# aj-prime/Elemental

Hardware: AMD Instinct MI355X
Metric: distributed Gemm TFLOP/s (fp64/fp32) at 1/2/4/8 GPUs; % of MFMA peak (higher is better)
Workload: dtype f64; 1 GPU; C2: El::Gemm NN f64 m=n=k=32768, Grid 1x1; m=32768, n=32768, k=32768, grid=1x1, algorithm=SUMMA_C, blocksize=128, compute_panel=auto, parallelism=grid1x1, comm_reserved_cus=0

## Files before the change

### elemental_amd/_lib.py

```python
from __future__ import annotations

import ctypes
import os
from ctypes import (CFUNCTYPE, POINTER, c_char_p, c_double, c_float, c_int, c_int64, c_size_t,
                    c_ubyte, c_uint16, c_uint64, c_void_p)

_HERE = os.path.dirname(os.path.abspath(__file__))
LIB_PATH = os.path.join(_HERE, "libelemental_amd.so")

OK, ERR_LOGIC, ERR_HIP, ERR_COMM, ERR_RUNTIME, ERR_UNSUPPORTED, ERR_NO_DEVICE, ERR_SINGULAR = range(8)
ERR_NOT_HPD = 8
NORMAL, TRANSPOSE, ADJOINT = 0, 1, 2
MC, MD, MR, VC, VR, STAR, CIRC = range(7)
(GEMM_DEFAULT, GEMM_SUMMA_A_MS, GEMM_SUMMA_A, GEMM_SUMMA_B_MS, GEMM_SUMMA_B, GEMM_SUMMA_C_MS,
 GEMM_SUMMA_C, GEMM_SUMMA_DOT, GEMM_CANNON) = range(9)
ROW_MAJOR, COLUMN_MAJOR = 0, 1
LOWER, UPPER = 0, 1
LEFT, RIGHT = 0, 1
NON_UNIT, UNIT = 0, 1
CPU, GPU = 0, 1
F32, F64, F16, BF16 = 0, 1, 2, 3
I32, I64, U8 = 4, 5, 6
OP_SUM, OP_PROD, OP_MAX, OP_MIN = 0, 1, 2, 3
(MAP_IDENTITY, MAP_NEGATE, MAP_ABS, MAP_SQUARE, MAP_SQRT, MAP_EXP, MAP_LOG, MAP_RELU, MAP_SIGMOID,
# ... 11 lines not shown
    "elx_last_error": (c_char_p, []),
    "elx_last_nonhpd_column": (_i, []),
    "elx_version": (_i, []),
    "elx_device_count": (_i, [POINTER(c_int)]),
    "elx_set_device": (_i, [_i]),
    "elx_get_device": (_i, [POINTER(c_int)]),
    "elx_device_synchronize": (_i, []),
    "elx_default_stream": (_i, [POINTER(c_void_p)]),
    "elx_comm_stream": (_i, [POINTER(c_void_p)]),
    "elx_reserved_cus": (_i, [POINTER(c_int)]),
    "elx_stream_create": (_i, [POINTER(c_void_p)]),
    "elx_stream_destroy": (_i, [_vp]),
    "elx_stream_synchronize": (_i, [_vp]),
    "elx_default_event": (_i, [POINTER(c_void_p)]),
    "elx_event_create": (_i, [POINTER(c_void_p)]),
    "elx_event_destroy": (_i, [_vp]),
    "elx_event_record": (_i, [_vp, _vp]),
    "elx_stream_wait_event": (_i, [_vp, _vp]),
    "elx_event_synchronize": (_i, [_vp]),
    "elx_pool_alloc": (_i, [POINTER(c_void_p), c_size_t, _vp]),
    "elx_pool_free": (_i, [_vp, _vp]),
    "elx_pool_trim": (_i, [c_size_t]),
    "elx_pool_stats": (_i, [POINTER(c_size_t), POINTER(c_size_t)]),
    "elx_pool_set_max_cached": (_i, [c_size_t]),
    "elx_pool_max_cached": (_i, [POINTER(c_size_t)]),
    "elx_pool_bin_bytes": (c_size_t, [c_size_t]),
    "elx_pool_bin_cacheable": (_i, [c_size_t]),
    "elx_pool_backing_reserved": (_i, [POINTER(c_size_t)]),
    "elx_memcpy_h2d": (_i, [_vp, _vp, c_size_t, _vp]),
    "elx_memcpy_d2h": (_i, [_vp, _vp, c_size_t, _vp]),
    "elx_memcpy_d2d": (_i, [_vp, _vp, c_size_t, _vp]),
    "elx_gemm_f64": (_i, [_i, _i, _i64, _i64, _i64, _d, _vp, _i64, _vp, _i64, _d, _vp, _i64, _vp]),
    "elx_gemm_f32": (_i, [_i, _i, _i64, _i64, _i64, c_float, _vp, _i64, _vp, _i64, c_float, _vp, _i64, _vp]),
    "elx_gemm_f16": (_i, [_i, _i, _i64, _i64, _i64, c_float, _vp, _i64, _vp, _i64, c_float, _vp, _i64, _vp]),
    "elx_gemm_bf16": (_i, [_i, _i, _i64, _i64, _i64, c_float, _vp, _i64, _vp, _i64, c_float, _vp, _i64, _vp]),
    "elx_matrix_gemm": (_i, [_i, _i, _i, _i, _i64, _i64, _i64, _d, _vp, _i64, _vp, _i64, _d, _vp, _i64, _vp]),
    "elx_matrix_fill": (_i, [_i, _i, _i64, _i64, _d, _vp, _i64, _vp]),
    "elx_matrix_scale": (_i, [_i, _i, _i64, _i64, _d, _vp, _i64, _vp]),
    "elx_matrix_axpy": (_i, [_i, _i, _i64, _i64, _d, _vp, _i64, _vp, _i64, _vp]),
    "elx_matrix_copy": (_i, [_i, _i, _i64, _i64, _vp, _i64, _vp, _i64, _vp]),
    "elx_matrix_trmm": (_i, [_i, _i, _i, _i, _i, _i, _i64, _i64, _d, _vp, _i64, _vp, _i64, _vp]),
    "elx_matrix_trsm": (_i, [_i, _i, _i, _i, _i, _i, _i64, _i64, _d, _vp, _i64, _vp, _i64, _vp]),
    "elx_trsm_plan": (_i, [_i, _i64, _i64, POINTER(c_int), POINTER(c_int), POINTER(c_int64)]),
    "elx_trsm_last_launch": (_i, []),
    "elx_matrix_cholesky": (_i, [_i, _i, _i, _i64, _vp, _i64, _vp]),
    "elx_matrix_triangular_inverse": (_i, [_i, _i, _i, _i, _i64, _vp, _i64, _vp]),
    "elx_matrix_trtrmm": (_i, [_i, _i, _i, _i64, _vp, _i64, _vp]),
    "elx_matrix_hpd_inverse": (_i, [_i, _i, _i, _i64, _vp, _i64, _vp]),
    "elx_matrix_lu": (_i, [_i, _i, _i64, _i64, _vp, _i64, _vp, _vp]),
    "elx_matrix_qr": (_i, [_i, _i, _i64, _i64, _vp, _i64, _vp, _vp, _vp]),
    "elx_matrix_hermitian_tridiag": (_i, [_i, _i, _i, _i64, _vp, _i64, _vp, _vp]),
    "elx_axpy2d": (_i, [_i, _i64, _i64, _d, _vp, _i64, _i64, _vp, _i64, _i64, _vp]),
    "elx_copy2d": (_i, [_i, _i64, _i64, _vp, _i64, _i64, _vp, _i64, _i64, _vp]),
    "elx_pack_strided": (_i, [_i, _i, _i64, _i64, _i64, _i64, _i64, _i64, _vp, _i64, _vp, _i64, _vp]),
    "elx_unpack_strided": (_i, [_i, _i, _i64, _i64, _i64, _i64, _i64, _i64, _vp, _i64, _vp, _i64, _vp]),
    "elx_pack_partial_strided": (_i, [_i, _i, _i, _i64, _i64, _i64, _i64, _i64, _i64, _i64, _i64, _vp, _i64, _vp,
                                      _i64, _vp]),
    "elx_unpack_partial_strided": (_i, [_i, _i, _i, _i64, _i64, _i64, _i64, _i64, _i64, _i64, _i64, _vp, _i64,
                                        _vp, _i64, _vp]),
    "elx_unpack_axpy_strided": (_i, [_i, _i, _i64, _i64, _d, _i64, _i64, _i64, _i64, _vp, _i64, _vp, _i64, _vp]),
    "elx_copy2d_convert": (_i, [_i, _i, _i64, _i64, _vp, _i64, _i64, _vp, _i64, _i64, _vp]),
    "elx_transpose": (_i, [_i, _i64, _i64, _vp, _i64, _vp, _i64, _vp]),
    "elx_scale2d": (_i, [_i, _i64, _i64, _d, _vp, _i64, _vp]),
    "elx_fill2d": (_i, [_i, _i64, _i64, _d, _vp, _i64, _vp]),
    "elx_hadamard2d": (_i, [_i, _i64, _i64, _vp, _i64, _vp, _i64, _vp, _i64, _vp]),
    "elx_entrywise_map": (_i, [_i, _i, _i64, _i64, _vp, _i64, _vp, _i64, _vp]),
# ... 214 lines not shown
```

### elemental_amd/csrc/capi.cpp

```cpp
#include "common.hpp"
#include "runtime/runtime.hpp"
#include "comm/comm.hpp"
#include "core/distmatrix.hpp"
#include "core/redist.hpp"
#include "core/gemm.hpp"
#include "core/level2.hpp"
#include "core/lu.hpp"
#include "core/qr.hpp"
#include "core/tridiag.hpp"
#include "core/random.hpp"
#include "core/io.hpp"
#include "core/exec.hpp"
#include <functional>
#include <string>

struct elx_comm_s { std::shared_ptr<elx::Comm> c; };
struct elx_grid_s { std::shared_ptr<elx::Grid> g; };
struct elx_dm_s { std::shared_ptr<elx::DistMatrix> m; };
struct elx_perm_s { elx::Permutation p; };

namespace elx {
namespace {
thread_local std::string g_last_error;

// ... 124 lines not shown
}
int elx_memcpy_d2h(void* dst, const void* src, size_t bytes, void* stream) {
    return Guard([&] {
        hipStream_t s = S(stream);
        ELX_CHECK_HIP(hipMemcpyAsync(dst, src, bytes, hipMemcpyDeviceToHost, s));
        ELX_CHECK_HIP(hipStreamSynchronize(s));
    });
}
int elx_memcpy_d2d(void* dst, const void* src, size_t bytes, void* stream) {
    return Guard([&] { ELX_CHECK_HIP(hipMemcpyAsync(dst, src, bytes, hipMemcpyDeviceToDevice, S(stream))); });
}

#define ELX_GEMM_ENTRY(NAME, DT, ST, SC)                                                              \
    int NAME(int opA, int opB, int64_t m, int64_t n, int64_t k, SC alpha, const ST* A, int64_t lda,    \
             const ST* B, int64_t ldb, SC beta, ST* C, int64_t ldc, void* stream) {                  \
        return Guard([&] {                                                                             \
            CheckOp(opA);                                                                              \
            CheckOp(opB);                                                                              \
            ELX_REQUIRE(m >= 0 && n >= 0 && k >= 0, "negative GEMM dimension");                       \
            const bool ta = opA != ELX_NORMAL, tb = opB != ELX_NORMAL;                                 \
            ELX_REQUIRE(ldc >= (m > 1 ? m : 1), "ldc too small");                                     \
            ELX_REQUIRE(lda >= ((ta ? k : m) > 1 ? (ta ? k : m) : 1), "lda too small");               \
            ELX_REQUIRE(ldb >= ((tb ? n : k) > 1 ? (tb ? n : k) : 1), "ldb too small");               \
            if (m == 0 || n == 0) return;                                                              \
            exec::Gemm(Device::GPU, DT, ta, tb, m, n, k, (double)alpha, A, lda, B, ldb, (double)beta, C, \
                       ldc, S(stream));                                                                \
        });                                                                                            \
    }
ELX_GEMM_ENTRY(elx_gemm_f64, DType::F64, double, double)
ELX_GEMM_ENTRY(elx_gemm_f32, DType::F32, float, float)
ELX_GEMM_ENTRY(elx_gemm_f16, DType::F16, uint16_t, float)
ELX_GEMM_ENTRY(elx_gemm_bf16, DType::BF16, uint16_t, float)
#undef ELX_GEMM_ENTRY

namespace {
hipStream_t DevStream(Device d, void* stream) { return d == Device::GPU ? S(stream) : nullptr; }
void CheckLd(int64_t ld, int64_t rows, const char* what) {
    ELX_REQUIRE(ld >= (rows > 1 ? rows : 1), what, " leading dimension ", ld, " < ", rows);
}
}
int elx_matrix_gemm(int dtype, int device, int opA, int opB, int64_t m, int64_t n, int64_t k, double alpha,
                    const void* A, int64_t lda, const void* B, int64_t ldb, double beta, void* C, int64_t ldc,
                    void* stream) {
    return Guard([&] {
        CheckOp(opA);
        CheckOp(opB);
        ELX_REQUIRE(m >= 0 && n >= 0 && k >= 0, "negative GEMM dimension");
        const bool ta = opA != ELX_NORMAL, tb = opB != ELX_NORMAL;
        CheckLd(ldc, m, "C");
        CheckLd(lda, ta ? k : m, "A");
        CheckLd(ldb, tb ? n : k, "B");
        if (m == 0 || n == 0) return;
        const Device d = ToDevice(device);
        if (k == 0) {
            if (beta == 0.0) exec::Fill(d, ToDType(dtype), m, n, 0.0, C, ldc, DevStream(d, stream));
            else if (beta != 1.0) exec::Scale(d, ToDType(dtype), m, n, beta, C, ldc, DevStream(d, stream));
            return;
        }
        exec::Gemm(d, ToDType(dtype), ta, tb, m, n, k, alpha, A, lda, B, ldb, beta, C, ldc, DevStream(d, stream));
    });
}
int elx_matrix_fill(int dtype, int device, int64_t m, int64_t n, double value, void* A, int64_t lda, void* stream) {
    return Guard([&] {
        CheckLd(lda, m, "A");
        if (m == 0 || n == 0) return;
        const Device d = ToDevice(device);
// ... 972 lines not shown
```

### elemental_amd/csrc/core/exec.cpp

```cpp
#include <cstdlib>
#include "exec.hpp"
#include "host_blas.hpp"
#include "host_leaves.hpp"
#include <cmath>
#include <type_traits>
#include <vector>

namespace elx {
namespace exec {

namespace {

[[noreturn]] void NotAMatrixType(DType t) { throw LogicError(Cat("dtype ", DTypeName(t), " is not a matrix type")); }
#define EXEC_SWITCH(t, T, ...) ELX_DTYPE_SWITCH(t, T, NotAMatrixType(t), __VA_ARGS__)
#define EXEC_REAL_SWITCH(t, T, ...) ELX_REAL_SWITCH(t, T, NotAMatrixType(t), __VA_ARGS__)

void check(hipError_t e, const char* what) {
    if (e != hipSuccess)
        throw HIPError(Cat(what, ": ", hipGetErrorName(e), " (", hipGetErrorString(e), ")"));
}

}

int CommCopyWGs() {
    static const int v = [] { const char* e = getenv("ELX_COMM_COPY_WGS"); return e ? atoi(e) : 256; }();
    return v;
}

void Copy2DBatch(Device dev, DType t, const Copy2D* d, int nd, bool axpy, double alpha, hipStream_t s) {
    if (nd <= 0) return;
    if (dev == Device::GPU) {
        const int cap = s != nullptr && s == Runtime::Get().CommStream() ? CommCopyWGs() : 0;
        check(kern::copy2d_batch(static_cast<int>(t), d, nd, axpy, alpha, s, cap), "copy2d_batch");
        return;
// ... 5 lines not shown
                 int nsrc, double alpha, hipStream_t s) {
    if (m <= 0 || n <= 0 || nsrc <= 0) return;
    if (dev == Device::GPU) {
        const int cap = s != nullptr && s == Runtime::Get().CommStream() ? CommCopyWGs() : 0;
        for (int q0 = 0; q0 < nsrc; q0 += kern::kMaxContractSources) {
            kern::ContractSum c{};
            c.m = m; c.n = n; c.dst = dst; c.dcs = dcs; c.drs = drs;
            c.nsrc = std::min(nsrc - q0, kern::kMaxContractSources);
            for (int q = 0; q < c.nsrc; ++q) {
                c.src[q] = src[q0 + q].p;
                c.scs[q] = src[q0 + q].cs;
                c.srs[q] = src[q0 + q].rs;
            }
            check(kern::contract_sum(static_cast<int>(t), c, alpha, s, cap), "contract_sum");
        }
        return;
    }
    for (int q = 0; q < nsrc; ++q) {
        const Copy2D d{m, n, src[q].p, src[q].cs, src[q].rs, dst, dcs, drs};
        EXEC_SWITCH(t, T, cpu_copy<T>(d, true, alpha));
    }
}

void Convert2D(Device dev, DType src_t, DType dst_t, const Copy2D& d, hipStream_t s) {
    if (d.m <= 0 || d.n <= 0) return;
    if (src_t == dst_t) { Copy2DBatch(dev, src_t, &d, 1, false, 0.0, s); return; }
    if (dev == Device::GPU) {
        check(kern::convert2d(static_cast<int>(src_t), static_cast<int>(dst_t), d, s), "convert2d");
        return;
    }
    EXEC_SWITCH(src_t, TS, EXEC_SWITCH(dst_t, TD, cpu_convert<TS, TD>(d)));
}

void Gemm(Device dev, DType t, bool ta, bool tb, Int m, Int n, Int k, double alpha, const void* A, Int lda,
          const void* B, Int ldb, double beta, void* C, Int ldc, hipStream_t s) {
    if (m <= 0 || n <= 0) return;
    if (dev == Device::GPU) {
        hipError_t e = hipSuccess;
        switch (t) {
        case DType::F64:
            e = kern::gemm_mfma<double>(ta, tb, m, n, k, alpha, static_cast<const double*>(A), lda,
                                        static_cast<const double*>(B), ldb, beta, static_cast<double*>(C), ldc, s);
            break;
        case DType::F32:
            e = kern::gemm_mfma<float>(ta, tb, m, n, k, (float)alpha, static_cast<const float*>(A), lda,
                                       static_cast<const float*>(B), ldb, (float)beta, static_cast<float*>(C),
                                       ldc, s);
            break;
        case DType::F16:
        case DType::BF16:
            e = kern::gemm_mfma_h(t == DType::BF16, ta, tb, m, n, k, (float)alpha,
                                  static_cast<const uint16_t*>(A), lda, static_cast<const uint16_t*>(B), ldb,
                                  (float)beta, static_cast<uint16_t*>(C), ldc, s);
            break;
        default:
            NotAMatrixType(t);
        }
        check(e, "gemm_mfma");
        return;
    }
    EXEC_SWITCH(t, T,
        cpu_gemm<T>(ta, tb, m, n, k, alpha, static_cast<const Stor<T>*>(A), lda, static_cast<const Stor<T>*>(B), ldb,
                    beta, static_cast<Stor<T>*>(C), ldc));
}

void Fill(Device dev, DType t, Int m, Int n, double v, void* A, Int lda, hipStream_t s) {
    if (m <= 0 || n <= 0) return;
    if (dev == Device::GPU) { check(kern::fill2d((int)t, m, n, v, A, lda, s), "fill2d"); return; }
// ... 390 lines not shown
```

### elemental_amd/csrc/core/exec.hpp

```cpp
#pragma once
#include "../common.hpp"
#include "../runtime/runtime.hpp"
#include "../kernels/kernels.hpp"

namespace elx {
namespace exec {

using kern::Copy2D;

void Copy2DBatch(Device dev, DType t, const Copy2D* d, int nd, bool axpy, double alpha, hipStream_t s);
struct ContractSource { const void* p; Int cs, rs; };
void ContractSum(Device dev, DType t, Int m, Int n, void* dst, Int dcs, Int drs, const ContractSource* src,
                 int nsrc, double alpha, hipStream_t s);
void Convert2D(Device dev, DType src_t, DType dst_t, const Copy2D& d, hipStream_t s);
void Gemm(Device dev, DType t, bool ta, bool tb, Int m, Int n, Int k, double alpha,
          const void* A, Int lda, const void* B, Int ldb, double beta, void* C, Int ldc, hipStream_t s);
void Fill(Device dev, DType t, Int m, Int n, double v, void* A, Int lda, hipStream_t s);
void Scale(Device dev, DType t, Int m, Int n, double alpha, void* A, Int lda, hipStream_t s);
double AbsMax(Device dev, DType t, Int m, Int n, const void* A, Int lda, hipStream_t s);
double ScaledSumSq(Device dev, DType t, Int m, Int n, const void* A, Int lda, double scale, hipStream_t s);
void Hadamard(Device dev, DType t, Int m, Int n, const void* A, Int lda, const void* B, Int ldb,
              void* C, Int ldc, hipStream_t s);
void Map(Device dev, DType t, int fn, Int m, Int n, const void* A, Int lda, void* B, Int ldb, hipStream_t s);
void Combine(Device dev, DType t, int fn, Int m, Int n, const void* A, Int lda, void* B, Int ldb, hipStream_t s);
void Trapezoid(Device dev, DType t, bool lower, Int m, Int n, double alpha, const void* X, Int ldx, double beta,
               void* Y, Int ldy, Int i0, Int is, Int j0, Int js, Int offset, hipStream_t s);
void Trsm(Device dev, DType t, bool lower, bool trans, bool unit, Int m, Int n, const void* A, Int lda, void* B,
          Int ldb, hipStream_t s);
void Trmm(Device dev, DType t, bool lower, bool trans, bool unit, Int m, Int n, double alpha, const void* A, Int lda,
          void* B, Int ldb, hipStream_t s);
void Cholesky(Device dev, DType t, bool lower, Int n, void* A, Int lda, int* info, int col0, hipStream_t s);
size_t LUWorkBytes(Device dev, Int m);
void LU(Device dev, DType t, Int m, Int w, void* A, Int lda, int* piv, int row_off, void* work, int* info, int col0,
        hipStream_t s);
void Laswp(Device dev, DType t, Int m, Int n, void* A, Int lda, const int* piv, Int k0, Int k1, Int voff, bool inverse,
           const int* info, hipStream_t s);
size_t QRWorkBytes(Device dev, Int m);
void QR(Device dev, DType t, Int m, Int w, void* A, Int lda, void* tau, void* sig, void* work, hipStream_t s);
void QRExplicitU(Device dev, DType t, Int m, Int nb, const void* A, Int lda, void* U, Int ldu, hipStream_t s,
                 bool upper = false, Int off = 0);
size_t SytrdWorkBytes(Int n);
void SytrdPanel(DType t, bool lower, Int n, Int c0, Int w, void* A, Int lda, void* tau, void* V, void* W, Int ldv,
                void* work, hipStream_t s);
void HostHermitianTridiag(DType t, bool lower, Int n, void* A, Int lda, void* tau);
void QRFixT(Device dev, DType t, Int nb, void* S, Int lds, const void* tau, hipStream_t s);
void RowScale(Device dev, DType t, Int m, Int n, void* A, Int lda, const void* sig, Int i0, Int is, hipStream_t s);
void TriangularInverse(Device dev, DType t, bool lower, bool unit, Int n, void* A, Int lda, hipStream_t s);
void Trtrmm(Device dev, DType t, bool lower, Int n, void* A, Int lda, hipStream_t s);
void TriInverseBatched(DType t, bool lower, bool trans, bool unit, Int nb, Int m, const void* A, Int lda, void* W,
// ... 22 lines not shown
```

### elemental_amd/csrc/kernels/blas1.hip

```cpp
#include <hip/hip_runtime.h>
#include "kernels.hpp"
#include "dtype_switch.hpp"
#include <algorithm>
#include <cstdlib>
#include <initializer_list>
#include <utility>

namespace elx {
namespace kern {

namespace {

constexpr int TILE = 64;
constexpr int NT = 256;
constexpr int UNROLL = 4;

struct CopyBatch {
    Copy2D d[kMaxCopyBatch];
};

template <typename S>
struct V16 {
    static constexpr int N = 16 / sizeof(S);
    S v[N];
// ... 453 lines not shown
                      [&](const S(&x)[2]) { return E::store(apply_combine(FN, E::load(x[1]), E::load(x[0]))); });
}

template <typename T>
__global__ __launch_bounds__(NT) void hash_kernel(i64 m, i64 n, typename Elem<T>::storage* A, i64 lda, i64 i0,
                                                  i64 istride, i64 j0, i64 jstride, uint64_t seed,
                                                  double center, double radius) {
    using E = Elem<T>;
    for_each_2d(m, n, [&](i64 i, i64 j) {
#pragma clang fp contract(off)
        const double u = hash_unit(seed, i0 + i * istride, j0 + j * jstride);
        const double v = center + radius * (2.0 * u - 1.0);
        A[i + j * lda] = E::store((typename E::compute)v);
    });
}

template <typename T>
__global__ __launch_bounds__(NT) void trapezoid_kernel(bool lower, i64 m, i64 n, double alpha,
                                                       const typename Elem<T>::storage* X, i64 ldx, double beta,
                                                       typename Elem<T>::storage* Y, i64 ldy, i64 i0, i64 istride,
                                                       i64 j0, i64 jstride, i64 offset) {
    using E = Elem<T>;
    using Cm = typename E::compute;
    const Cm a = (Cm)alpha, b = (Cm)beta;
    for_each_2d(m, n, [&](i64 i, i64 j) {
        const i64 gi = i0 + i * istride, gj = j0 + j * jstride - offset;
        if (lower ? gi < gj : gi > gj) return;
        Cm y = (X && beta == 0.0) ? Cm(0) : b * E::load(Y[i + j * ldy]);
        if (X) y = y + a * E::load(X[i + j * ldx]);
        Y[i + j * ldy] = E::store(y);
    });
}

struct EwShape {
    i64 m, n;
    bool vec;
    dim3 grid;
};
template <typename S>
EwShape ew_shape(i64 m, i64 n, std::initializer_list<std::pair<const void*, i64>> ops) {
    bool contig = true, vec = true;
    for (auto& o : ops) {
        contig = contig && (o.second == m || n == 1);
        vec = vec && (reinterpret_cast<uintptr_t>(o.first) % 16 == 0);
    }
    if (contig) { m *= n; n = 1; }
    for (auto& o : ops) vec = vec && (n == 1 || (o.second * (i64)sizeof(S)) % 16 == 0);
    constexpr int N = 16 / sizeof(S);
    i64 gx = (m + (i64)NT * N * UNROLL - 1) / ((i64)NT * N * UNROLL);
    const i64 gy = n < 1 ? 1 : (n > 65535 ? 65535 : n);
    gx = std::max<i64>(1, std::min<i64>(gx, (1ll << 31) - 1));
    return EwShape{m, n, vec, dim3((unsigned)gx, (unsigned)gy)};
}

dim3 grid2d(i64 m, i64 n) {
    i64 gx = (m + NT - 1) / NT;
    if (gx > 64) gx = 64;
    if (gx < 1) gx = 1;
    i64 gy = n < 1 ? 1 : n;
    if (gy > 4096) gy = 4096;
    return dim3((unsigned)gx, (unsigned)gy);
}

bool TransposeVec(const Copy2D& x, int es) {
    const bool src_i = x.scs == 1, dst_i = x.dcs == 1;
    if (src_i == dst_i || (src_i ? false : x.srs != 1) || (dst_i ? false : x.drs != 1)) return false;
// ... 203 lines not shown
hipError_t combine(int dtype, int fn, i64 m, i64 n, const void* A, i64 lda, void* B, i64 ldb, hipStream_t s) {
    if (m <= 0 || n <= 0) return hipSuccess;
#define ELX_COMBINE_CASE(F) case F: launch_combine<T, F>(s, m, n, A, lda, B, ldb); break;
    ELX_KERN_SWITCH(dtype, T, switch (fn) {
        ELX_COMBINE_CASE(ELX_COMBINE_ADD) ELX_COMBINE_CASE(ELX_COMBINE_SUB) ELX_COMBINE_CASE(ELX_COMBINE_MUL)
        ELX_COMBINE_CASE(ELX_COMBINE_DIV) ELX_COMBINE_CASE(ELX_COMBINE_MAX) ELX_COMBINE_CASE(ELX_COMBINE_MIN)
        ELX_COMBINE_CASE(ELX_COMBINE_RELU_GRAD)
        default: return hipErrorInvalidValue;
    });
#undef ELX_COMBINE_CASE
    return hipGetLastError();
}

hipError_t fill_hash(int dtype, i64 m, i64 n, void* A, i64 lda, i64 i0, i64 istride, i64 j0, i64 jstride,
                     uint64_t seed, double center, double radius, hipStream_t s) {
    if (m <= 0 || n <= 0) return hipSuccess;
    ELX_KERN_SWITCH(dtype, T,
        hipLaunchKernelGGL((hash_kernel<T>), grid2d(m, n), dim3(NT), 0, s, m, n,
                           static_cast<typename Elem<T>::storage*>(A), lda, i0, istride, j0, jstride,
                           seed, center, radius));
    return hipGetLastError();
}

hipError_t trapezoid2d(int dtype, bool lower, i64 m, i64 n, double alpha, const void* X, i64 ldx, double beta,
                       void* Y, i64 ldy, i64 i0, i64 istride, i64 j0, i64 jstride, i64 offset, hipStream_t s) {
    if (m <= 0 || n <= 0) return hipSuccess;
    ELX_KERN_SWITCH(dtype, T,
        hipLaunchKernelGGL((trapezoid_kernel<T>), grid2d(m, n), dim3(NT), 0, s, lower, m, n, alpha,
                           static_cast<const typename Elem<T>::storage*>(X), ldx, beta,
                           static_cast<typename Elem<T>::storage*>(Y), ldy, i0, istride, j0, jstride, offset));
    return hipGetLastError();
}

}
}
```

### elemental_amd/csrc/kernels/kernels.hpp

```cpp
#pragma once
#include <hip/hip_runtime.h>
#include <algorithm>
#include <cstdint>
#include <cstdlib>

namespace elx {
namespace kern {

hipError_t workspace_alloc(void** p, size_t bytes, hipStream_t s);
hipError_t workspace_free(void* p, hipStream_t s);

using i64 = int64_t;

template <typename T>
hipError_t gemm_mfma(bool ta, bool tb, i64 m, i64 n, i64 k, T alpha, const T* A, i64 lda,
                     const T* B, i64 ldb, T beta, T* C, i64 ldc, hipStream_t s);
struct DmaPlan {
    bool use;
    i64 kmain, kchunk;
    int nz;
};
inline DmaPlan dma_plan(bool ok, i64 tiles, i64 k, int bk, i64 slots = 512) {
    DmaPlan d{false, 0, 0, 1};
    if (!ok) return d;
// ... 85 lines not shown
        const i64 z = std::min<i64>(std::min<i64>((256 + tiles - 1) / tiles, kmain / (min_kt * BK)), split_cap);
        if (z >= 2) {
            pl.kchunk = ((kmain + z - 1) / z + BK - 1) / BK * BK;
            pl.nz = (kmain + pl.kchunk - 1) / pl.kchunk;
        }
    }
    return pl;
}

hipError_t gemm_mfma_h(bool is_bf16, bool ta, bool tb, i64 m, i64 n, i64 k, float alpha,
                       const uint16_t* A, i64 lda, const uint16_t* B, i64 ldb, float beta,
                       uint16_t* C, i64 ldc, hipStream_t s);
hipError_t gemm_mfma_h_simple(bool is_bf16, bool ta, bool tb, i64 m, i64 n, i64 k, float alpha,
                              const uint16_t* A, i64 lda, const uint16_t* B, i64 ldb, float beta,
                              uint16_t* C, i64 ldc, hipStream_t s);

struct Copy2D {
    i64 m, n;
    const void* src; i64 scs, srs;
    void* dst; i64 dcs, drs;
};
constexpr int kMaxCopyBatch = 16;
hipError_t copy2d_batch(int dtype, const Copy2D* d, int nd, bool axpy, double alpha, hipStream_t s, int max_wgs = 0);

constexpr int kMaxContractSources = 16;
struct ContractSum {
    i64 m, n;
    void* dst; i64 dcs, drs;
    int nsrc;
    const void* src[kMaxContractSources];
    i64 scs[kMaxContractSources], srs[kMaxContractSources];
};
hipError_t contract_sum(int dtype, const ContractSum& c, double alpha, hipStream_t s, int max_wgs = 0);

hipError_t convert2d(int src_dtype, int dst_dtype, const Copy2D& d, hipStream_t s);
hipError_t fill2d(int dtype, i64 m, i64 n, double v, void* A, i64 lda, hipStream_t s);
constexpr int kNormPartsMax = 4096;
hipError_t norm_partials(int dtype, int mode, i64 m, i64 n, const void* A, i64 lda, double scale, double* out,
                         int* nparts, hipStream_t s);
hipError_t scale2d(int dtype, i64 m, i64 n, double alpha, void* A, i64 lda, hipStream_t s);
hipError_t hadamard2d(int dtype, i64 m, i64 n, const void* A, i64 lda, const void* B, i64 ldb,
                      void* C, i64 ldc, hipStream_t s);
hipError_t entrywise_map(int dtype, int fn, i64 m, i64 n, const void* A, i64 lda, void* B, i64 ldb,
                         hipStream_t s);
hipError_t combine(int dtype, int fn, i64 m, i64 n, const void* A, i64 lda, void* B, i64 ldb, hipStream_t s);
hipError_t fill_hash(int dtype, i64 m, i64 n, void* A, i64 lda, i64 i0, i64 istride, i64 j0,
                     i64 jstride, uint64_t seed, double center, double radius, hipStream_t s);

hipError_t trapezoid2d(int dtype, bool lower, i64 m, i64 n, double alpha, const void* X, i64 ldx, double beta,
                       void* Y, i64 ldy, i64 i0, i64 istride, i64 j0, i64 jstride, i64 offset, hipStream_t s);
hipError_t trsm_local(int dtype, bool ident, bool lower, bool trans, bool unit, i64 m, i64 n, const void* A, i64 lda,
                      void* B, i64 ldb, hipStream_t s);
constexpr long kTriInverseLdsMax = 150 * 1024;
bool tri_inverse_lds_ok(int dtype, i64 nb);
hipError_t tri_inverse_batched(int dtype, bool lower, bool trans, bool unit, i64 nb, i64 m, const void* A, i64 lda,
                               void* W, hipStream_t s);
constexpr i64 kTrsmInvertMaxRows = 256;
constexpr long kTrsmLdsMax = 66 * 1024;
struct TrsmPlan { bool invert; bool lds; size_t lds_bytes; };
constexpr TrsmPlan trsm_plan(size_t es, i64 m, i64 n) {
    const size_t bytes = (size_t)m * 65 * es;
    return TrsmPlan{m <= kTrsmInvertMaxRows && n >= 4 * m, bytes <= (size_t)kTrsmLdsMax, bytes};
}
constexpr bool trsm_batched_ok(size_t es, i64 nb, i64 m, i64 local_width) {
    return nb * 65 * (i64)es <= kTriInverseLdsMax && (m + nb - 1) / nb <= 65535 && local_width >= 4 * nb;
}
// ... 51 lines not shown
```

### include/elemental_amd.h

```cpp
#ifndef ELEMENTAL_AMD_H
#define ELEMENTAL_AMD_H

#include <stddef.h>
#include <stdint.h>

#ifdef __cplusplus
extern "C" {
#endif

#define ELX_OK                  0
#define ELX_ERR_LOGIC           1
#define ELX_ERR_HIP             2
#define ELX_ERR_COMM            3
#define ELX_ERR_RUNTIME         4
#define ELX_ERR_UNSUPPORTED     5
#define ELX_ERR_NO_DEVICE       6
#define ELX_ERR_SINGULAR        7
#define ELX_ERR_NOT_HPD         8

#define ELX_NORMAL     0
#define ELX_TRANSPOSE  1
#define ELX_ADJOINT    2
#define ELX_MC    0
#define ELX_MD    1
// ... 58 lines not shown
int elx_comm_stream(void** stream);
int elx_reserved_cus(int* cus);
int elx_stream_create(void** stream);
int elx_stream_destroy(void* stream);
int elx_stream_synchronize(void* stream);
int elx_default_event(void** event);
int elx_event_create(void** event);
int elx_event_destroy(void* event);
int elx_event_record(void* event, void* stream);
int elx_stream_wait_event(void* stream, void* event);
int elx_event_synchronize(void* event);

int elx_pool_alloc(void** ptr, size_t bytes, void* stream);
int elx_pool_free(void* ptr, void* stream);
int elx_pool_trim(size_t bytes_to_keep);
int elx_pool_stats(size_t* bytes_reserved, size_t* bytes_in_use);
int elx_pool_set_max_cached(size_t bytes);
int elx_pool_max_cached(size_t* bytes);
size_t elx_pool_bin_bytes(size_t bytes);
int elx_pool_bin_cacheable(size_t bytes);
int elx_pool_backing_reserved(size_t* bytes);
int elx_memcpy_h2d(void* dst, const void* src, size_t bytes, void* stream);
int elx_memcpy_d2h(void* dst, const void* src, size_t bytes, void* stream);
int elx_memcpy_d2d(void* dst, const void* src, size_t bytes, void* stream);

int elx_gemm_f64(int opA, int opB, int64_t m, int64_t n, int64_t k,
                 double alpha, const double* A, int64_t lda,
                 const double* B, int64_t ldb,
                 double beta, double* C, int64_t ldc, void* stream);
int elx_gemm_f32(int opA, int opB, int64_t m, int64_t n, int64_t k,
                 float alpha, const float* A, int64_t lda,
                 const float* B, int64_t ldb,
                 float beta, float* C, int64_t ldc, void* stream);
int elx_gemm_f16(int opA, int opB, int64_t m, int64_t n, int64_t k,
                 float alpha, const uint16_t* A, int64_t lda,
                 const uint16_t* B, int64_t ldb,
                 float beta, uint16_t* C, int64_t ldc, void* stream);
int elx_gemm_bf16(int opA, int opB, int64_t m, int64_t n, int64_t k,
                  float alpha, const uint16_t* A, int64_t lda,
                  const uint16_t* B, int64_t ldb,
                  float beta, uint16_t* C, int64_t ldc, void* stream);

int elx_matrix_gemm(int dtype, int device, int opA, int opB, int64_t m, int64_t n, int64_t k,
                    double alpha, const void* A, int64_t lda, const void* B, int64_t ldb,
                    double beta, void* C, int64_t ldc, void* stream);
int elx_matrix_fill(int dtype, int device, int64_t m, int64_t n, double value,
                    void* A, int64_t lda, void* stream);
int elx_matrix_scale(int dtype, int device, int64_t m, int64_t n, double alpha,
                     void* A, int64_t lda, void* stream);
int elx_matrix_axpy(int dtype, int device, int64_t m, int64_t n, double alpha,
                    const void* X, int64_t ldx, void* Y, int64_t ldy, void* stream);
int elx_matrix_copy(int dtype, int device, int64_t m, int64_t n, const void* A, int64_t lda,
                    void* B, int64_t ldb, void* stream);
int elx_matrix_trmm(int dtype, int device, int side, int uplo, int orient, int diag,
                    int64_t m, int64_t n, double alpha, const void* A, int64_t lda,
                    void* B, int64_t ldb, void* stream);
int elx_matrix_trsm(int dtype, int device, int side, int uplo, int orient, int diag,
                    int64_t m, int64_t n, double alpha, const void* A, int64_t lda,
                    void* B, int64_t ldb, void* stream);
int elx_trsm_plan(int dtype, int64_t m, int64_t n, int* invert, int* lds, int64_t* lds_bytes);
int elx_trsm_last_launch(void);
int elx_matrix_cholesky(int dtype, int device, int uplo, int64_t n, void* A, int64_t lda, void* stream);
int elx_matrix_triangular_inverse(int dtype, int device, int uplo, int diag, int64_t n, void* A, int64_t lda,
                                  void* stream);
int elx_matrix_trtrmm(int dtype, int device, int uplo, int64_t n, void* A, int64_t lda, void* stream);
int elx_matrix_hpd_inverse(int dtype, int device, int uplo, int64_t n, void* A, int64_t lda, void* stream);
// ... 256 lines not shown
```

Before: 76.32 TFLOP/s.

## Add one-level Strassen recursion for large f32/f64 GEMMs

Routes eligible f32/f64 GEMMs (all dims even and at least 8192, nonzero alpha, GPU) through a Strassen-Winograd recursion, one level by default and configurable via environment variables. It replaces eight half-size multiplies with seven, plus new fused quadrant-sum and quadrant-scatter kernels. The aim is to cut MFMA work by about one eighth in exchange for extra memory-bound additions, three half-size workspace buffers, and weaker floating-point error bounds compared with classical GEMM.

New measurement: 86.03 TFLOP/s, median of 6. +12.7%, better.

```diff
diff --git a/elemental_amd/_lib.py b/elemental_amd/_lib.py
--- a/elemental_amd/_lib.py
+++ b/elemental_amd/_lib.py
@@ -67,6 +67,7 @@
     "elx_memcpy_d2d": (_i, [_vp, _vp, c_size_t, _vp]),
     "elx_gemm_f64": (_i, [_i, _i, _i64, _i64, _i64, _d, _vp, _i64, _vp, _i64, _d, _vp, _i64, _vp]),
     "elx_gemm_f32": (_i, [_i, _i, _i64, _i64, _i64, c_float, _vp, _i64, _vp, _i64, c_float, _vp, _i64, _vp]),
+    "elx_gemm_last_levels": (_i, []),
     "elx_gemm_f16": (_i, [_i, _i, _i64, _i64, _i64, c_float, _vp, _i64, _vp, _i64, c_float, _vp, _i64, _vp]),
     "elx_gemm_bf16": (_i, [_i, _i, _i64, _i64, _i64, c_float, _vp, _i64, _vp, _i64, c_float, _vp, _i64, _vp]),
     "elx_matrix_gemm": (_i, [_i, _i, _i, _i, _i64, _i64, _i64, _d, _vp, _i64, _vp, _i64, _d, _vp, _i64, _vp]),
diff --git a/elemental_amd/csrc/capi.cpp b/elemental_amd/csrc/capi.cpp
--- a/elemental_amd/csrc/capi.cpp
+++ b/elemental_amd/csrc/capi.cpp
@@ -180,6 +180,7 @@
 ELX_GEMM_ENTRY(elx_gemm_f16, DType::F16, uint16_t, float)
 ELX_GEMM_ENTRY(elx_gemm_bf16, DType::BF16, uint16_t, float)
 #undef ELX_GEMM_ENTRY
+int elx_gemm_last_levels(void) { return exec::GemmLastLevels(); }
 
 namespace {
 hipStream_t DevStream(Device d, void* stream) { return d == Device::GPU ? S(stream) : nullptr; }
diff --git a/elemental_amd/csrc/core/exec.cpp b/elemental_amd/csrc/core/exec.cpp
--- a/elemental_amd/csrc/core/exec.cpp
+++ b/elemental_amd/csrc/core/exec.cpp
@@ -1,5 +1,6 @@
 #include <cstdlib>
 #include "exec.hpp"
+#include "strassen.hpp"
 #include "host_blas.hpp"
 #include "host_leaves.hpp"
 #include <cmath>
@@ -71,8 +72,56 @@
     EXEC_SWITCH(src_t, TS, EXEC_SWITCH(dst_t, TD, cpu_convert<TS, TD>(d)));
 }
 
+namespace {
+thread_local int t_gemm_levels = 0;
+}
+int GemmLastLevels() { return t_gemm_levels; }
+
 void Gemm(Device dev, DType t, bool ta, bool tb, Int m, Int n, Int k, double alpha, const void* A, Int lda,
           const void* B, Int ldb, double beta, void* C, Int ldc, hipStream_t s) {
+    t_gemm_levels = 0;
+    if (m <= 0 || n <= 0) return;
+    if (k >= 2 && (t == DType::F64 || t == DType::F32)) {
+        const strassen::Knobs kn = strassen::ReadKnobs();
+        t_gemm_levels = strassen::Gemm(kn.levels, kn, dev, t, ta, tb, m, n, k, alpha, A, lda, B, ldb, beta, C, ldc, s);
+        if (t_gemm_levels > 0) return;
+    }
+    GemmPlain(dev, t, ta, tb, m, n, k, alpha, A, lda, B, ldb, beta, C, ldc, s);
+}
+
+void QuadSum(Device dev, DType t, const kern::QuadSum* q, int nq, hipStream_t s) {
+    RequireReal(t, "QuadSum");
+    if (dev == Device::GPU) { check(kern::quad_sum((int)t, q, nq, s), "quad_sum"); return; }
+    for (int d = 0; d < nq; ++d)
+        EXEC_REAL_SWITCH(t, T, {
+            const kern::QuadSum& a = q[d];
+            const T* x = static_cast<const T*>(a.x);
+            const T* y = static_cast<const T*>(a.y);
+            T* o = static_cast<T*>(a.d);
+            for (Int j = 0; j < a.n; ++j)
+                for (Int i = 0; i < a.m; ++i) o[i + j * a.ldd] = x[i + j * a.ldx] + (T)a.sy * y[i + j * a.ldy];
+        });
+}
+
+void QuadScatter(Device dev, DType t, const kern::QuadScatter& q, hipStream_t s) {
+    RequireReal(t, "QuadScatter");
+    if (dev == Device::GPU) { check(kern::quad_scatter((int)t, q, s), "quad_scatter"); return; }
+    EXEC_REAL_SWITCH(t, T, {
+        const T* M = static_cast<const T*>(q.M);
+        for (int w = 0; w < q.nt; ++w) {
+            T* c = static_cast<T*>(q.c[w]);
+            for (Int j = 0; j < q.n; ++j)
+                for (Int i = 0; i < q.m; ++i) {
+                    T v = (T)q.coef[w] * M[i + j * q.ldm];
+                    if (q.beta[w] != 0.0) v = v + (T)q.beta[w] * c[i + j * q.ldc[w]];
+                    c[i + j * q.ldc[w]] = v;
+                }
+        }
+    });
+}
+
+void GemmPlain(Device dev, DType t, bool ta, bool tb, Int m, Int n, Int k, double alpha, const void* A, Int lda,
+               const void* B, Int ldb, double beta, void* C, Int ldc, hipStream_t s) {
     if (m <= 0 || n <= 0) return;
     if (dev == Device::GPU) {
         hipError_t e = hipSuccess;
diff --git a/elemental_amd/csrc/core/exec.hpp b/elemental_amd/csrc/core/exec.hpp
--- a/elemental_amd/csrc/core/exec.hpp
+++ b/elemental_amd/csrc/core/exec.hpp
@@ -15,6 +15,11 @@
 void Convert2D(Device dev, DType src_t, DType dst_t, const Copy2D& d, hipStream_t s);
 void Gemm(Device dev, DType t, bool ta, bool tb, Int m, Int n, Int k, double alpha,
           const void* A, Int lda, const void* B, Int ldb, double beta, void* C, Int ldc, hipStream_t s);
+void GemmPlain(Device dev, DType t, bool ta, bool tb, Int m, Int n, Int k, double alpha,
+               const void* A, Int lda, const void* B, Int ldb, double beta, void* C, Int ldc, hipStream_t s);
+int GemmLastLevels();
+void QuadSum(Device dev, DType t, const kern::QuadSum* q, int nq, hipStream_t s);
+void QuadScatter(Device dev, DType t, const kern::QuadScatter& q, hipStream_t s);
 void Fill(Device dev, DType t, Int m, Int n, double v, void* A, Int lda, hipStream_t s);
 void Scale(Device dev, DType t, Int m, Int n, double alpha, void* A, Int lda, hipStream_t s);
 double AbsMax(Device dev, DType t, Int m, Int n, const void* A, Int lda, hipStream_t s);
diff --git a/elemental_amd/csrc/core/strassen.cpp b/elemental_amd/csrc/core/strassen.cpp
--- /dev/null
+++ b/elemental_amd/csrc/core/strassen.cpp
@@ -0,0 +1,107 @@
+#include "strassen.hpp"
+#include "exec.hpp"
+#include <cstdlib>
+
+namespace elx {
+namespace strassen {
+
+Knobs ReadKnobs() {
+    Knobs kn{1, kDefaultMin, false};
+    if (const char* v = getenv("ELX_GEMM_STRASSEN")) kn.levels = std::max(0, std::min(2, atoi(v)));
+    if (const char* v = getenv("ELX_GEMM_STRASSEN_MIN")) {
+        kn.min = std::max<Int>(2, atoll(v));
+        kn.forced = true;
+    }
+    return kn;
+}
+
+bool Eligible(Device dev, DType t, Int m, Int n, Int k, double alpha, const Knobs& kn) {
+    if (t != DType::F64 && t != DType::F32) return false;
+    if (dev != Device::GPU && !kn.forced) return false;
+    if ((m | n | k) & 1) return false;
+    return std::min(m, std::min(n, k)) >= kn.min && alpha != 0.0;
+}
+
+namespace {
+
+struct Work {
+    Device dev;
+    hipStream_t s;
+    void* p = nullptr;
+    Work(Device d, hipStream_t st) : dev(d), s(st) {}
+    Work(const Work&) = delete;
+    Work& operator=(const Work&) = delete;
+    bool Alloc(size_t bytes) {
+        if (dev == Device::GPU) return kern::workspace_alloc(&p, bytes, s) == hipSuccess && p != nullptr;
+        p = std::malloc(bytes);
+        return p != nullptr;
+    }
+    ~Work() {
+        if (!p) return;
+        if (dev == Device::GPU) (void)kern::workspace_free(p, s);
+        else std::free(p);
+    }
+};
+
+int Multiply(int levels, const Knobs& kn, Device dev, DType t, bool ta, bool tb, Int m, Int n, Int k, double alpha,
+             const void* A, Int lda, const void* B, Int ldb, double beta, void* C, Int ldc, hipStream_t s) {
+    const int used = Gemm(levels, kn, dev, t, ta, tb, m, n, k, alpha, A, lda, B, ldb, beta, C, ldc, s);
+    if (used == 0) exec::GemmPlain(dev, t, ta, tb, m, n, k, alpha, A, lda, B, ldb, beta, C, ldc, s);
+    return used;
+}
+
+}
+
+int Gemm(int levels, const Knobs& kn, Device dev, DType t, bool ta, bool tb, Int m, Int n, Int k, double alpha,
+         const void* A, Int lda, const void* B, Int ldb, double beta, void* C, Int ldc, hipStream_t s) {
+    if (levels <= 0 || !Eligible(dev, t, m, n, k, alpha, kn)) return 0;
+    const Int m2 = m / 2, n2 = n / 2, k2 = k / 2;
+    const size_t es = DTypeSize(t);
+    const Int ra = ta ? k2 : m2, ca = ta ? m2 : k2, rb = tb ? n2 : k2, cb = tb ? k2 : n2;
+    Work Sw(dev, s), Tw(dev, s), Mw(dev, s);
+    if (!Sw.Alloc((size_t)ra * ca * es) || !Tw.Alloc((size_t)rb * cb * es) || !Mw.Alloc((size_t)m2 * n2 * es)) return 0;
+    void* S = Sw.p;
+    void* T = Tw.p;
+    void* M = Mw.p;
+
+    const char* a = static_cast<const char*>(A);
+    const char* b = static_cast<const char*>(B);
+    char* c = static_cast<char*>(C);
+    auto Aq = [&](int p, int q) -> const void* { return a + (ta ? q * k2 + p * m2 * lda : p * m2 + q * k2 * lda) * (Int)es; };
+    auto Bq = [&](int p, int q) -> const void* { return b + (tb ? q * n2 + p * k2 * ldb : p * k2 + q * n2 * ldb) * (Int)es; };
+    auto Cq = [&](int p, int q) -> void* { return c + (p * m2 + q * n2 * ldc) * (Int)es; };
+
+    auto sums = [&](const void* X, Int ldx, const void* Y, Int ldy, double sx, const void* V, Int ldv, const void* W,
+                    Int ldw, double sv) {
+        const kern::QuadSum q[2] = {{ra, ca, S, ra, X, ldx, Y, ldy, sx}, {rb, cb, T, rb, V, ldv, W, ldw, sv}};
+        exec::QuadSum(dev, t, q, 2, s);
+    };
+    auto scatter = [&](int nt, void* c0, double beta0, void* c1, double beta1) {
+        const kern::QuadScatter q{m2, n2, M, m2, nt, {c0, c1}, {ldc, ldc}, {beta0, beta1}, {alpha, alpha}};
+        exec::QuadScatter(dev, t, q, s);
+    };
+    int deep = 0;
+    auto mul = [&](double al, const void* X, Int ldx, const void* Y, Int ldy, double be, void* Z, Int ldz) {
+        deep = std::max(deep, Multiply(levels - 1, kn, dev, t, ta, tb, m2, n2, k2, al, X, ldx, Y, ldy, be, Z, ldz, s));
+    };
+
+    sums(Aq(1, 0), lda, Aq(1, 1), lda, 1.0, Bq(0, 1), ldb, Bq(0, 0), ldb, -1.0);
+    mul(1.0, S, ra, T, rb, 0.0, M, m2);
+    scatter(2, Cq(0, 1), beta, Cq(1, 1), beta);
+    sums(S, ra, Aq(0, 0), lda, -1.0, Bq(1, 1), ldb, T, rb, -1.0);
+    mul(1.0, Aq(0, 0), lda, Bq(0, 0), ldb, 0.0, M, m2);
+    scatter(1, Cq(0, 0), beta, nullptr, 0.0);
+    mul(alpha, Aq(0, 1), lda, Bq(1, 0), ldb, 1.0, Cq(0, 0), ldc);
+    mul(1.0, S, ra, T, rb, 1.0, M, m2);
+    sums(Aq(0, 1), lda, S, ra, -1.0, T, rb, Bq(1, 0), ldb, -1.0);
+    mul(alpha, S, ra, Bq(1, 1), ldb, 1.0, Cq(0, 1), ldc);
+    mul(-alpha, Aq(1, 1), lda, T, rb, beta, Cq(1, 0), ldc);
+    scatter(1, Cq(0, 1), 1.0, nullptr, 0.0);
+    sums(Aq(0, 0), lda, Aq(1, 0), lda, -1.0, Bq(1, 1), ldb, Bq(0, 1), ldb, -1.0);
+    mul(1.0, S, ra, T, rb, 1.0, M, m2);
+    scatter(2, Cq(1, 0), 1.0, Cq(1, 1), 1.0);
+    return 1 + deep;
+}
+
+}
+}
diff --git a/elemental_amd/csrc/core/strassen.hpp b/elemental_amd/csrc/core/strassen.hpp
--- /dev/null
+++ b/elemental_amd/csrc/core/strassen.hpp
@@ -0,0 +1,24 @@
+#pragma once
+#include "../common.hpp"
+#include "../runtime/runtime.hpp"
+
+namespace elx {
+namespace strassen {
+
+constexpr Int kMinFloor = 8192;
+constexpr Int kDefaultMin = kMinFloor;
+
+struct Knobs {
+    int levels;
+    Int min;
+    bool forced;
+};
+Knobs ReadKnobs();
+
+bool Eligible(Device dev, DType t, Int m, Int n, Int k, double alpha, const Knobs& kn);
+
+int Gemm(int levels, const Knobs& kn, Device dev, DType t, bool ta, bool tb, Int m, Int n, Int k, double alpha,
+         const void* A, Int lda, const void* B, Int ldb, double beta, void* C, Int ldc, hipStream_t s);
+
+}
+}
diff --git a/elemental_amd/csrc/kernels/blas1.hip b/elemental_amd/csrc/kernels/blas1.hip
--- a/elemental_amd/csrc/kernels/blas1.hip
+++ b/elemental_amd/csrc/kernels/blas1.hip
@@ -509,6 +509,95 @@
     });
 }
 
+struct QuadSumBatch {
+    QuadSum q[2];
+};
+
+template <typename T>
+__global__ __launch_bounds__(NT) void quad_sum_kernel(QuadSumBatch b, bool vec) {
+    using E = Elem<T>;
+    using S = typename E::storage;
+    const QuadSum& q = b.q[blockIdx.z];
+    const auto sy = (typename E::compute)q.sy;
+    S* const p[3] = {static_cast<S*>(q.d), const_cast<S*>(static_cast<const S*>(q.x)),
+                     const_cast<S*>(static_cast<const S*>(q.y))};
+    const i64 l[3] = {q.ldd, q.ldx, q.ldy};
+    ew_2d<S, 3, false>(q.m, q.n, p, l, vec, [&](const S(&x)[3]) { return E::store(E::load(x[1]) + sy * E::load(x[2])); });
+}
+
+template <typename T>
+__global__ __launch_bounds__(NT) void quad_scatter_kernel(QuadScatter q, bool vec) {
+    using E = Elem<T>;
+    using S = typename E::storage;
+    using Cm = typename E::compute;
+    constexpr int N = V16<S>::N;
+    constexpr i64 CHUNK = (i64)NT * UNROLL * N;
+    const S* M = static_cast<const S*>(q.M);
+    S* const c0p = static_cast<S*>(q.c[0]);
+    S* const c1p = static_cast<S*>(q.c[1]);
+    const bool two = q.nt > 1;
+    const bool rd0 = q.beta[0] != 0.0, rd1 = two && q.beta[1] != 0.0;
+    const Cm b0 = (Cm)q.beta[0], b1 = (Cm)q.beta[1], a0 = (Cm)q.coef[0], a1 = (Cm)q.coef[1];
+    auto out = [](Cm a, S mv, bool rd, Cm b, S cv) {
+        Cm v = a * E::load(mv);
+        if (rd) v = v + b * E::load(cv);
+        return E::store(v);
+    };
+    for (i64 j = blockIdx.y; j < q.n; j += gridDim.y) {
+        const S* mc = M + j * q.ldm;
+        S* y0 = c0p + j * q.ldc[0];
+        S* y1 = two ? c1p + j * q.ldc[1] : nullptr;
+        for (i64 c0 = (i64)blockIdx.x * CHUNK; c0 < q.m; c0 += (i64)gridDim.x * CHUNK) {
+            if (vec && c0 + CHUNK <= q.m) {
+                V16<S> x[UNROLL], u0[UNROLL] = {}, u1[UNROLL] = {};
+#pragma unroll
+                for (int u = 0; u < UNROLL; ++u) {
+                    const i64 i = c0 + (u * NT + threadIdx.x) * N;
+                    x[u] = *reinterpret_cast<const V16<S>*>(mc + i);
+                    if (rd0) u0[u] = *reinterpret_cast<const V16<S>*>(y0 + i);
+                    if (rd1) u1[u] = *reinterpret_cast<const V16<S>*>(y1 + i);
+                }
+#pragma unroll
+                for (int u = 0; u < UNROLL; ++u) {
+                    const i64 i = c0 + (u * NT + threadIdx.x) * N;
+#pragma unroll
+                    for (int e = 0; e < N; ++e) u0[u].v[e] = out(a0, x[u].v[e], rd0, b0, u0[u].v[e]);
+                    *reinterpret_cast<V16<S>*>(y0 + i) = u0[u];
+                    if (two) {
+#pragma unroll
+                        for (int e = 0; e < N; ++e) u1[u].v[e] = out(a1, x[u].v[e], rd1, b1, u1[u].v[e]);
+                        *reinterpret_cast<V16<S>*>(y1 + i) = u1[u];
+                    }
+                }
+            } else {
+                const i64 end = c0 + CHUNK < q.m ? c0 + CHUNK : q.m;
+                for (i64 i = c0 + (i64)threadIdx.x * N; i < end; i += (i64)NT * N) {
+                    if (vec && i + N <= end) {
+                        const V16<S> x = *reinterpret_cast<const V16<S>*>(mc + i);
+                        V16<S> u0 = {}, u1 = {};
+                        if (rd0) u0 = *reinterpret_cast<const V16<S>*>(y0 + i);
+                        if (rd1) u1 = *reinterpret_cast<const V16<S>*>(y1 + i);
+#pragma unroll
+                        for (int e = 0; e < N; ++e) u0.v[e] = out(a0, x.v[e], rd0, b0, u0.v[e]);
+                        *reinterpret_cast<V16<S>*>(y0 + i) = u0;
+                        if (two) {
+#pragma unroll
+                            for (int e = 0; e < N; ++e) u1.v[e] = out(a1, x.v[e], rd1, b1, u1.v[e]);
+                            *reinterpret_cast<V16<S>*>(y1 + i) = u1;
+                        }
+                    } else {
+                        for (i64 e = i; e < i + N && e < end; ++e) {
+                            const S mv = mc[e];
+                            y0[e] = out(a0, mv, rd0, b0, rd0 ? y0[e] : S{});
+                            if (two) y1[e] = out(a1, mv, rd1, b1, rd1 ? y1[e] : S{});
+                        }
+                    }
+                }
+            }
+        }
+    }
+}
+
 struct EwShape {
     i64 m, n;
     bool vec;
@@ -778,5 +867,49 @@
     return hipGetLastError();
 }
 
-}
-}
+namespace {
+template <typename S>
+dim3 quad_grid(i64 m, i64 n, int nz) {
+    constexpr i64 chunk = (i64)NT * UNROLL * (16 / sizeof(S));
+    const i64 gx = std::max<i64>(1, std::min<i64>((m + chunk - 1) / chunk, (1ll << 31) - 1));
+    return dim3((unsigned)gx, (unsigned)std::max<i64>(1, std::min<i64>(n, 65535)), (unsigned)nz);
+}
+bool quad_al16(const void* p, i64 ld, i64 n, int es) {
+    return reinterpret_cast<uintptr_t>(p) % 16 == 0 && (n == 1 || (ld * es) % 16 == 0);
+}
+}
+
+hipError_t quad_sum(int dtype, const QuadSum* q, int nq, hipStream_t s) {
+    if (nq < 1 || nq > 2) return hipErrorInvalidValue;
+    const int es = dtype_size(dtype);
+    QuadSumBatch b{};
+    i64 m = 0, n = 0;
+    int used = 0;
+    bool vec = true;
+    for (int i = 0; i < nq; ++i) {
+        if (q[i].m <= 0 || q[i].n <= 0) continue;
+        b.q[used++] = q[i];
+        m = std::max(m, q[i].m);
+        n = std::max(n, q[i].n);
+        vec = vec && quad_al16(q[i].d, q[i].ldd, q[i].n, es) && quad_al16(q[i].x, q[i].ldx, q[i].n, es) &&
+              quad_al16(q[i].y, q[i].ldy, q[i].n, es);
+    }
+    if (used == 0) return hipSuccess;
+    ELX_KERN_REAL_SWITCH(dtype, T,
+        hipLaunchKernelGGL((quad_sum_kernel<T>), quad_grid<T>(m, n, used), dim3(NT), 0, s, b, vec));
+    return hipGetLastError();
+}
+
+hipError_t quad_scatter(int dtype, const QuadScatter& q, hipStream_t s) {
+    if (q.nt < 1 || q.nt > 2) return hipErrorInvalidValue;
+    if (q.m <= 0 || q.n <= 0) return hipSuccess;
+    const int es = dtype_size(dtype);
+    bool vec = quad_al16(q.M, q.ldm, q.n, es);
+    for (int t = 0; t < q.nt; ++t) vec = vec && quad_al16(q.c[t], q.ldc[t], q.n, es);
+    ELX_KERN_REAL_SWITCH(dtype, T,
+        hipLaunchKernelGGL((quad_scatter_kernel<T>), quad_grid<T>(q.m, q.n, 1), dim3(NT), 0, s, q, vec));
+    return hipGetLastError();
+}
+
+}
+}
diff --git a/elemental_amd/csrc/kernels/kernels.hpp b/elemental_amd/csrc/kernels/kernels.hpp
--- a/elemental_amd/csrc/kernels/kernels.hpp
+++ b/elemental_amd/csrc/kernels/kernels.hpp
@@ -141,6 +141,23 @@
     i64 scs[kMaxContractSources], srs[kMaxContractSources];
 };
 hipError_t contract_sum(int dtype, const ContractSum& c, double alpha, hipStream_t s, int max_wgs = 0);
+
+struct QuadSum {
+    i64 m, n;
+    void* d; i64 ldd;
+    const void* x; i64 ldx;
+    const void* y; i64 ldy;
+    double sy;
+};
+struct QuadScatter {
+    i64 m, n;
+    const void* M; i64 ldm;
+    int nt;
+    void* c[2]; i64 ldc[2];
+    double beta[2], coef[2];
+};
+hipError_t quad_sum(int dtype, const QuadSum* q, int nq, hipStream_t s);
+hipError_t quad_scatter(int dtype, const QuadScatter& q, hipStream_t s);
 
 hipError_t convert2d(int src_dtype, int dst_dtype, const Copy2D& d, hipStream_t s);
 hipError_t fill2d(int dtype, i64 m, i64 n, double v, void* A, i64 lda, hipStream_t s);
diff --git a/include/elemental_amd.h b/include/elemental_amd.h
--- a/include/elemental_amd.h
+++ b/include/elemental_amd.h
@@ -114,6 +114,7 @@
                  float alpha, const float* A, int64_t lda,
                  const float* B, int64_t ldb,
                  float beta, float* C, int64_t ldc, void* stream);
+int elx_gemm_last_levels(void);
 int elx_gemm_f16(int opA, int opB, int64_t m, int64_t n, int64_t k,
                  float alpha, const uint16_t* A, int64_t lda,
                  const uint16_t* B, int64_t ldb,
```
